# batra-mlp-lab/visdial

Measured on AMD Instinct MI355X. Metric: QA-rounds/sec training mn-att-ques-im-hist+disc (batch 20x10x100), higher is better.
Workload: dtype f32 operands and results; the option recurrence multiplies the EXACT 3-way bf16 split of both operands (9 bf16 MFMA products per fp32 product, f32 accumulate: fp32-grade, errors at the f32 MFMA's own level) -- its two step kernels and its weight-gradient contraction; f32 MFMA (v_mfma_f32_32x32x2_f32

## Files before the change

### visdial_amd/csrc/gemm_core.h

```cpp
#pragma once
#include <stdint.h>
#include <stdlib.h>
#include <type_traits>

#include "common.h"

#ifdef VD_TIMING
#define VD_TSLOTS 12
#define VD_TBLOCKS 8192
static __device__ unsigned long long vd_tbuf[VD_TBLOCKS * VD_TSLOTS];
#define VD_TSTAMP(i, clk)                                                                \
  do {                                                                                   \
    if (threadIdx.x == 0 && blockIdx.x < VD_TBLOCKS) vd_tbuf[blockIdx.x * VD_TSLOTS + (i)] = (clk); \
  } while (0)
#define VD_T(i) VD_TSTAMP(i, __builtin_amdgcn_s_memtime())
#define VD_TREAL(i) VD_TSTAMP(i, __builtin_amdgcn_s_memrealtime())
#else
#define VD_T(i) do {} while (0)
#define VD_TREAL(i) do {} while (0)
#endif

template <int WM_, int WK_, int NT_, int KW_, int DB_ = 1, int MINW_ = 1, int LDSMIN_ = 0, int BF16_ = 0>
struct GemmCfg {
  static constexpr int WM = WM_, WK = WK_, NT = NT_, KW = KW_, DB = DB_, MINW = MINW_;
  static constexpr int BM = WM * 32, BN = NT * 32, BK = WK * KW;
  static constexpr int THREADS = WM * WK * 64;
  static constexpr int BF16 = BF16_;
  static constexpr int ELEM_BYTES = BF16 ? 2 : 4;
  static constexpr int STRIDE = BF16 ? BK + 8 : BK + 4;
  static constexpr int BUF_FLOATS = (BM + BN) * STRIDE;
  static constexpr int STAGE_BYTES = (DB == 1 ? 2 : 1) * BUF_FLOATS * ELEM_BYTES;
  static constexpr int RED_BYTES = (WK - 1) * WM * 16 * 64 * 4;
  static constexpr int EPI_BYTES = WM * 32 * 32 * 4;
  static constexpr int LDS_BYTES0 = STAGE_BYTES > RED_BYTES ? STAGE_BYTES : RED_BYTES;
  static constexpr int LDS_BYTES1 = LDS_BYTES0 > EPI_BYTES ? LDS_BYTES0 : EPI_BYTES;
  static constexpr int LDS_BYTES = LDS_BYTES1 > LDSMIN_ ? LDS_BYTES1 : LDSMIN_;
  static constexpr int NA = (BM * BK / 4) / THREADS;
  static constexpr int NB = (BN * BK / 4) / THREADS;
  static_assert(KW % 8 == 0, "KW must be a multiple of 8");
  static_assert(!BF16 || (KW % 16 == 0 && DB == 0), "bf16 tiles: 16 k per MFMA, single-buffer pipeline only");
  static_assert((BM * BK / 4) % THREADS == 0 && NA >= 1, "A tile must split evenly");
  static_assert((BN * BK / 4) % THREADS == 0 && NB >= 1, "B tile must split evenly");
  static_assert(LDS_BYTES <= 160 * 1024, "LDS budget");
};

struct SrcRow {
  static constexpr bool KMAJOR = false;
  static constexpr bool PLAIN = true;
  const float* p;
  long ld;
  __device__ __forceinline__ const float* ptr(int r, int k) const { return p + (long)r * ld + k; }
  __device__ __forceinline__ long kstep() const { return 1; }
  __device__ __forceinline__ float4 ld4(int r, int k) const {
    return *reinterpret_cast<const float4*>(p + (long)r * ld + k);
  }
};
struct SrcK {
  static constexpr bool KMAJOR = true;
  static constexpr bool PLAIN = true;
  const float* p;
  long ld;
  __device__ __forceinline__ const float* ptr(int r, int k) const { return p + (long)k * ld + r; }
  __device__ __forceinline__ long kstep() const { return ld; }
  __device__ __forceinline__ float4 ld4(int r, int k) const {
    return *reinterpret_cast<const float4*>(p + (long)k * ld + r);
  }
};
struct SrcKRows {
  static constexpr bool KMAJOR = true;
  static constexpr bool PLAIN = false;
  const float* p;
  long ld;
  const int* rows;
  __device__ __forceinline__ float4 ld4(int r, int k) const {
    return *reinterpret_cast<const float4*>(p + (long)rows[k] * ld + r);
  }
};
struct SrcKGate4 {
  static constexpr bool KMAJOR = true;
  static constexpr bool PLAIN = true;
  const float* p;
  long ld;
  int H;
  __device__ __forceinline__ const float* ptr(int vc, int k) const {
    const int jb = vc >> 7, g = (vc >> 5) & 3, jj = vc & 31;
    return p + (long)k * ld + g * H + jb * 32 + jj;
  }
  __device__ __forceinline__ long kstep() const { return ld; }
  __device__ __forceinline__ float4 ld4(int vc, int k) const {
    const int jb = vc >> 7, g = (vc >> 5) & 3, jj = vc & 31;
    return *reinterpret_cast<const float4*>(p + (long)k * ld + g * H + jb * 32 + jj);
  }
};

__device__ __forceinline__ int mfma_row(int r, int lane) {
  return (r & 3) + 8 * (r >> 2) + 4 * (lane >> 5);
}

__device__ __forceinline__ void tile_to_rows(const f32x16& a, float* scr, int lane, float4 (&out)[4]) {
  asm volatile("" ::: "memory");
#pragma unroll
  for (int r = 0; r < 16; ++r) scr[mfma_row(r, lane) * 32 + (lane & 31)] = a[r];
  asm volatile("" ::: "memory");
#pragma unroll
  for (int p = 0; p < 4; ++p)
    out[p] = *reinterpret_cast<const float4*>(scr + (p * 8 + (lane >> 3)) * 32 + (lane & 7) * 4);
  asm volatile("" ::: "memory");
}

struct EpiNoPre {};
template <class Epi, class = void>
struct EpiPreOf {
  static constexpr bool value = false;
  using type = EpiNoPre;
};
template <class Epi>
struct EpiPreOf<Epi, std::void_t<typename Epi::Pre>> {
  static constexpr bool value = true;
  using type = typename Epi::Pre;
};

template <class Epi, class = void>
struct EpiDistOf {
  static constexpr bool value = false;
};
template <class Epi>
struct EpiDistOf<Epi, std::void_t<typename Epi::DOps>> {
  static constexpr bool value = Epi::HAS_DIST;
};

template <class Epi, class = void>
struct EpiDeadOf {
  static constexpr bool value = false;
};
template <class Epi>
struct EpiDeadOf<Epi, std::void_t<decltype(Epi::HAS_DEAD)>> {
  static constexpr bool value = Epi::HAS_DEAD;
};

template <class Epi, class = void>
struct EpiARowsOf {
  static constexpr bool value = false;
};
template <class Epi>
struct EpiARowsOf<Epi, std::void_t<decltype(Epi::HAS_AROWS)>> {
  static constexpr bool value = Epi::HAS_AROWS;
};

__device__ __forceinline__ void live_tile(int bid, int tiles_n, int& tile_m, int& tile_n) {
  const int li = bid >> 3;
  tile_m = (li / tiles_n) * 8 + (bid & 7);
  tile_n = li % tiles_n;
}

__device__ __forceinline__ int xcd_remap(int bid, int nwg) {
  const int q = nwg >> 3, r = nwg & 7;
  const int xcd = bid & 7, li = bid >> 3;
  const int base = xcd < r ? xcd * (q + 1) : r * (q + 1) + (xcd - r) * q;
  return base + li;
}

template <int D, int BK>
__device__ __forceinline__ void kmaj_piece(int f, int& r4, int& kk) {
  if constexpr (BK % 16 == 0) {
    const int klo = f & 15, g = f >> 4;
    r4 = g % (D / 4);
    kk = (g / (D / 4)) * 16 + klo;
    return;
  }
  const int klo = f & 7, g = f >> 3;
  r4 = g % (D / 4);
  kk = (g / (D / 4)) * 8 + klo;
}

template <class Cfg, class ASrc, class BSrc, class Epi>
__device__ __forceinline__ void gemm_block(int M, int N, int ks, int ke, int row_base, int col_base, int rot_seed,
                                           const ASrc& asrc, const BSrc& bsrc, const Epi& epi, float* smem,
                                           int tid_in = -1) {
  constexpr int WM = Cfg::WM, NT = Cfg::NT, KW = Cfg::KW;
  constexpr int BM = Cfg::BM, BN = Cfg::BN, BK = Cfg::BK;
  constexpr int THREADS = Cfg::THREADS, STR = Cfg::STRIDE;
  constexpr int NA = Cfg::NA, NB = Cfg::NB;
  const int tid = tid_in >= 0 ? tid_in : (int)threadIdx.x, lane = tid & 63, wave = tid >> 6;
  const int wm = wave % WM, wk = wave / WM;
  const int nk = ke > ks ? (ke - ks + BK - 1) / BK : 0;

  VD_T(0);
  VD_TREAL(6);
  f32x16 acc[NT];
#pragma unroll
  for (int j = 0; j < NT; ++j)
#pragma unroll
    for (int r = 0; r < 16; ++r) acc[j][r] = 0.f;

  float4 ra[NA], rb[NB];
  float4 ra2[NA], rb2[NB];

  const float* pa[NA];
  const float* pb[NB];
  int ka[NA], kb[NB];
  if constexpr (ASrc::PLAIN) {
#pragma unroll
    for (int i = 0; i < NA; ++i) {
      const int f = tid + i * THREADS;
      int gr;
      if constexpr (!ASrc::KMAJOR) {
        gr = row_base + f / (BK / 4);
        ka[i] = (f % (BK / 4)) * 4;
      } else {
        int r4;
        kmaj_piece<BM, BK>(f, r4, ka[i]);
        gr = row_base + r4 * 4;
      }
      pa[i] = gr < M ? asrc.ptr(gr, ka[i]) : nullptr;
    }
  }
  if constexpr (BSrc::PLAIN) {
#pragma unroll
    for (int i = 0; i < NB; ++i) {
      const int f = tid + i * THREADS;
      int gr;
      if constexpr (!BSrc::KMAJOR) {
        gr = col_base + f / (BK / 4);
        kb[i] = (f % (BK / 4)) * 4;
      } else {
        int r4;
        kmaj_piece<BN, BK>(f, r4, kb[i]);
        gr = col_base + r4 * 4;
      }
      pb[i] = gr < N ? bsrc.ptr(gr, kb[i]) : nullptr;
    }
  }

  auto load_tile_into = [&](int k0, float4 (&ra)[NA], float4 (&rb)[NB]) {
    if constexpr (ASrc::PLAIN) {
      const long off = (long)k0 * asrc.kstep();
#pragma unroll
      for (int i = 0; i < NA; ++i)
        ra[i] = (pa[i] != nullptr && k0 + ka[i] < ke) ? *reinterpret_cast<const float4*>(pa[i] + off)
                                                      : make_float4(0.f, 0.f, 0.f, 0.f);
    } else {
#pragma unroll
    for (int i = 0; i < NA; ++i) {
      const int f = tid + i * THREADS;
      float4 v = make_float4(0.f, 0.f, 0.f, 0.f);
      if constexpr (!ASrc::KMAJOR) {
        const int r = f / (BK / 4), kq = f % (BK / 4);
        const int gr = row_base + r, gk = k0 + kq * 4;
        if (gr < M && gk < ke) v = asrc.ld4(gr, gk);
      } else {
        int r4, kk;
        kmaj_piece<BM, BK>(f, r4, kk);
        const int gr = row_base + r4 * 4, gk = k0 + kk;
        if (gr < M && gk < ke) v = asrc.ld4(gr, gk);
      }
      ra[i] = v;
    }
    }
    if constexpr (BSrc::PLAIN) {
      const long off = (long)k0 * bsrc.kstep();
#pragma unroll
      for (int i = 0; i < NB; ++i)
        rb[i] = (pb[i] != nullptr && k0 + kb[i] < ke) ? *reinterpret_cast<const float4*>(pb[i] + off)
                                                      : make_float4(0.f, 0.f, 0.f, 0.f);
    } else {
#pragma unroll
    for (int i = 0; i < NB; ++i) {
      const int f = tid + i * THREADS;
      float4 v = make_float4(0.f, 0.f, 0.f, 0.f);
      if constexpr (!BSrc::KMAJOR) {
        const int r = f / (BK / 4), kq = f % (BK / 4);
        const int gr = col_base + r, gk = k0 + kq * 4;
        if (gr < N && gk < ke) v = bsrc.ld4(gr, gk);
      } else {
        int r4, kk;
        kmaj_piece<BN, BK>(f, r4, kk);
        const int gr = col_base + r4 * 4, gk = k0 + kk;
        if (gr < N && gk < ke) v = bsrc.ld4(gr, gk);
      }
      rb[i] = v;
    }
    }
  };

  auto load_tile = [&](int k0) { load_tile_into(k0, ra, rb); };

  using elem_t = std::conditional_t<Cfg::BF16 != 0, __bf16, float>;
  typedef __bf16 bf16x4_t __attribute__((ext_vector_type(4)));
  typedef __bf16 bf16x8_t __attribute__((ext_vector_type(8)));
  elem_t* const smem_e = reinterpret_cast<elem_t*>(smem);
  auto put_row4 = [&](elem_t* d, const float4& v) {
    if constexpr (Cfg::BF16) {
      bf16x4_t t = {(__bf16)v.x, (__bf16)v.y, (__bf16)v.z, (__bf16)v.w};
      *reinterpret_cast<bf16x4_t*>(d) = t;
    } else {
      *reinterpret_cast<float4*>(d) = v;
    }
  };
  auto put_col4 = [&](elem_t* d, const float4& v) {
    d[0] = (elem_t)v.x;
    d[STR] = (elem_t)v.y;
    d[2 * STR] = (elem_t)v.z;
    d[3 * STR] = (elem_t)v.w;
  };
  auto store_tile_from = [&](int buf, const float4 (&ra)[NA], const float4 (&rb)[NB]) {
    elem_t* sa = smem_e + buf * Cfg::BUF_FLOATS;
    elem_t* sb = sa + BM * STR;
#pragma unroll
    for (int i = 0; i < NA; ++i) {
      const int f = tid + i * THREADS;
      if constexpr (!ASrc::KMAJOR) {
        const int r = f / (BK / 4), kq = f % (BK / 4);
        put_row4(sa + r * STR + kq * 4, ra[i]);
      } else {
        int r4, kk;
        kmaj_piece<BM, BK>(f, r4, kk);
        put_col4(sa + (r4 * 4) * STR + kk, ra[i]);
      }
    }
#pragma unroll
    for (int i = 0; i < NB; ++i) {
      const int f = tid + i * THREADS;
      if constexpr (!BSrc::KMAJOR) {
        const int r = f / (BK / 4), kq = f % (BK / 4);
        put_row4(sb + r * STR + kq * 4, rb[i]);
      } else {
        int r4, kk;
        kmaj_piece<BN, BK>(f, r4, kk);
        put_col4(sb + (r4 * 4) * STR + kk, rb[i]);
      }
    }
  };

  const int rot = (rot_seed >= 0 && nk > 1) ? rot_seed % nk : 0;
  auto ktile = [&](int kt) {
    int t = kt + rot;
    if (t >= nk) t -= nk;
    return ks + t * BK;
  };
  auto store_tile = [&](int buf) { store_tile_from(buf, ra, rb); };

  const int frag_off = (lane & 31) * STR + wk * KW + (lane >> 5) * (Cfg::BF16 ? 8 : 4);
  auto mfma_tile = [&](int buf) {
    const elem_t* sa = smem_e + buf * Cfg::BUF_FLOATS + (wm * 32) * STR + frag_off;
    const elem_t* sb = smem_e + buf * Cfg::BUF_FLOATS + BM * STR + frag_off;
    if constexpr (Cfg::BF16) {
#pragma unroll
      for (int kc = 0; kc < KW / 16; ++kc) {
        const bf16x8_t a8 = *reinterpret_cast<const bf16x8_t*>(sa + kc * 16);
        bf16x8_t b8[NT];
#pragma unroll
        for (int j = 0; j < NT; ++j) b8[j] = *reinterpret_cast<const bf16x8_t*>(sb + j * 32 * STR + kc * 16);
#pragma unroll
        for (int j = 0; j < NT; ++j) acc[j] = __builtin_amdgcn_mfma_f32_32x32x16_bf16(a8, b8[j], acc[j], 0, 0, 0);
      }
    } else {
#pragma unroll
      for (int kc = 0; kc < KW / 8; ++kc) {
        const float4 a4 = *reinterpret_cast<const float4*>(sa + kc * 8);
        float4 b4[NT];
#pragma unroll
        for (int j = 0; j < NT; ++j) b4[j] = *reinterpret_cast<const float4*>(sb + j * 32 * STR + kc * 8);
#pragma unroll
        for (int j = 0; j < NT; ++j) acc[j] = __builtin_amdgcn_mfma_f32_32x32x2f32(a4.x, b4[j].x, acc[j], 0, 0, 0);
#pragma unroll
        for (int j = 0; j < NT; ++j) acc[j] = __builtin_amdgcn_mfma_f32_32x32x2f32(a4.y, b4[j].y, acc[j], 0, 0, 0);
#pragma unroll
        for (int j = 0; j < NT; ++j) acc[j] = __builtin_amdgcn_mfma_f32_32x32x2f32(a4.z, b4[j].z, acc[j], 0, 0, 0);
#pragma unroll
        for (int j = 0; j < NT; ++j) acc[j] = __builtin_amdgcn_mfma_f32_32x32x2f32(a4.w, b4[j].w, acc[j], 0, 0, 0);
      }
    }
  };

  if constexpr (Cfg::DB == 2) {
    if (nk > 0) load_tile_into(ktile(0), ra, rb);
    if (nk > 1) load_tile_into(ktile(1), ra2, rb2);
    for (int kt = 0; kt < nk; kt += 2) {
      store_tile_from(0, ra, rb);
      __syncthreads();
      if (kt == 0) VD_T(1);
      if (kt + 2 < nk) load_tile_into(ktile(kt + 2), ra, rb);
      mfma_tile(0);
      __syncthreads();
      if (kt + 1 < nk) {
        store_tile_from(0, ra2, rb2);
        __syncthreads();
        if (kt + 3 < nk) load_tile_into(ktile(kt + 3), ra2, rb2);
        mfma_tile(0);
        __syncthreads();
      }
    }
    VD_T(2);
  } else if constexpr (Cfg::DB == 1) {
    if (nk > 0) {
      load_tile(ktile(0));
      store_tile(0);
    }
    __syncthreads();
    for (int kt = 0; kt < nk; ++kt) {
      const int cur = kt & 1;
      if (kt + 1 < nk) load_tile(ktile(kt + 1));
      mfma_tile(cur);
      if (kt + 1 < nk) store_tile(cur ^ 1);
      __syncthreads();
    }
  } else {
    if (nk > 0) load_tile(ktile(0));
    for (int kt = 0; kt < nk; ++kt) {
      store_tile(0);
// ... 658 lines not shown
```

### visdial_amd/csrc/split_core.h

```cpp
#pragma once
#include "gemm_core.h"
#include "paths.h"

typedef __bf16 vd_bf16x8 __attribute__((ext_vector_type(8)));
typedef float vd_f32x4 __attribute__((ext_vector_type(4)));

__device__ __forceinline__ void vd_split3(const float4& u, const float4& w, vd_bf16x8& hi, vd_bf16x8& mid, vd_bf16x8& lo) {
  const float v[8] = {u.x, u.y, u.z, u.w, w.x, w.y, w.z, w.w};
#pragma unroll
  for (int i = 0; i < 8; ++i) {
    const __bf16 h = (__bf16)v[i];
    const float r1 = v[i] - (float)h;
    const __bf16 m = (__bf16)r1;
    const float r2 = r1 - (float)m;
    hi[i] = h; mid[i] = m; lo[i] = (__bf16)r2;
  }
}

static __global__ void __launch_bounds__(256) f32_to_bf16x3_kernel(const float* __restrict__ src, vd_bf16_bits* __restrict__ dst, long n4, long plane) {
  const long i = (long)blockIdx.x * 256 + threadIdx.x;
  if (i >= n4) return;
  const float4 v = reinterpret_cast<const float4*>(src)[i];
  float4 r1, r2;
  typedef __bf16 bf4 __attribute__((ext_vector_type(4)));
  const bf4 h = {(__bf16)v.x, (__bf16)v.y, (__bf16)v.z, (__bf16)v.w};
  r1.x = v.x - (float)h[0]; r1.y = v.y - (float)h[1]; r1.z = v.z - (float)h[2]; r1.w = v.w - (float)h[3];
  const bf4 m = {(__bf16)r1.x, (__bf16)r1.y, (__bf16)r1.z, (__bf16)r1.w};
  r2.x = r1.x - (float)m[0]; r2.y = r1.y - (float)m[1]; r2.z = r1.z - (float)m[2]; r2.w = r1.w - (float)m[3];
  const bf4 l = {(__bf16)r2.x, (__bf16)r2.y, (__bf16)r2.z, (__bf16)r2.w};
  *reinterpret_cast<bf4*>(dst + i * 4) = h;
  *reinterpret_cast<bf4*>(dst + plane + i * 4) = m;
  *reinterpret_cast<bf4*>(dst + 2 * plane + i * 4) = l;
}
static int weights_to_bf16x3(const float* src, vd_bf16_bits* dst, long n, hipStream_t s) {
  hipLaunchKernelGGL(f32_to_bf16x3_kernel, dim3((unsigned)((n / 4 + 255) / 256)), dim3(256), 0, s, src, dst, n / 4, n);
  VD_LAUNCH_CHECK();
  return VD_OK;
}

struct SplitCfg {
  static constexpr int NT = 4, WM = 4, THREADS = 256;
  static constexpr int BM = 128, BN = 128;
  static constexpr int ATILE = BM * 64;
  static constexpr int BTILE = BN * 32;
  static constexpr int STAGE = ATILE + 3 * BTILE;
#ifndef VD_SPLIT_LDS
#define VD_SPLIT_LDS 41984
#endif
  static constexpr int LDS_BYTES = VD_SPLIT_LDS;
  static_assert(LDS_BYTES >= 2 * STAGE, "two stages of 20 KB");
};

#ifndef VD_SPLIT_CG
#define VD_SPLIT_CG 2
#endif
static_assert(VD_SPLIT_CG >= 1 && VD_SPLIT_CG <= 8 && 8 % VD_SPLIT_CG == 0, "the XCD grid is VD_SPLIT_CG x (8 / VD_SPLIT_CG)");
__device__ __forceinline__ bool split_tile_of(int bid, int nwg, int tiles_m, int tiles_n, int& tile_m, int& tile_n) {
  constexpr int CG = VD_SPLIT_CG, RG = 8 / CG;
  if ((tiles_n % CG) == 0 && tiles_n >= 8) {
    const int xcd = bid & 7, li = bid >> 3, cpg = tiles_n / CG, rpg = (tiles_m + RG - 1) / RG;
    tile_n = (xcd % CG) * cpg + li % cpg;
    tile_m = (xcd / CG) * rpg + li / cpg;
    return tile_m < tiles_m && li / cpg < rpg;
  }
  const int wg = xcd_remap(bid, nwg);
  tile_n = wg % tiles_n;
  tile_m = wg / tiles_n;
  return true;
}
static int split_grid(int tiles_m, int tiles_n) {
  constexpr int CG = VD_SPLIT_CG, RG = 8 / CG;
  if ((tiles_n % CG) == 0 && tiles_n >= 8) return 8 * ((tiles_m + RG - 1) / RG) * (tiles_n / CG);
  return tiles_m * tiles_n;
}

template <int NPROD, class Epi>
__global__ void __launch_bounds__(256, 3)
gemm_split_kernel(int M, int N, int K, int tiles_n, const float* A, long lda, const vd_bf16_bits* B, long ldb, long bplane, Epi epi) {
  using Cfg = SplitCfg;
  constexpr int NT = Cfg::NT;
  extern __shared__ __attribute__((aligned(16))) float smem[];
  int tile_m, tile_n;
  if (!split_tile_of((int)blockIdx.x, (int)gridDim.x, (M + Cfg::BM - 1) / Cfg::BM, tiles_n, tile_m, tile_n)) return;
  const int row_base = tile_m * Cfg::BM, col_base = tile_n * Cfg::BN;
  constexpr int NIA = 2;
  constexpr int NIB = 3;
  const int tid = (int)threadIdx.x, lane = tid & 63;
  const int wm = __builtin_amdgcn_readfirstlane(tid >> 6);
  const int nm = K / 16;
  const int wrow = row_base + wm * 32;

  f32x16 acc[NT];
#pragma unroll
  for (int j = 0; j < NT; ++j)
#pragma unroll
    for (int r = 0; r < 16; ++r) acc[j][r] = 0.f;

  typename EpiPreOf<Epi>::type pre;
  if constexpr (EpiPreOf<Epi>::value) epi.preload(pre, wrow, lane, M);

  unsigned voffa[NIA], voffb[NIB];
#pragma unroll
  for (int i = 0; i < NIA; ++i) {
    const int r = wm * 32 + i * 16 + (lane >> 2);
    const int c = (lane & 3) ^ ((r >> 2) & 3);
    voffa[i] = (unsigned)(((long)min(row_base + r, M - 1) * lda + c * 4) * 4);
  }
  {
    const int r = wm * 32 + (lane >> 1);
    const int c = (lane & 1) ^ ((r >> 4) & 1);
    const unsigned v = (unsigned)(((long)min(col_base + r, N - 1) * ldb + c * 8) * 2);
#pragma unroll
    for (int i = 0; i < NIB; ++i) voffb[i] = v;
  }
  const unsigned lds0 = (unsigned)(uintptr_t)smem;
  auto issue = [&](int m, int st) {
    const unsigned base = lds0 + st * Cfg::STAGE;
#pragma unroll
    for (int i = 0; i < NIB; ++i)
      glds16(voffb[i], reinterpret_cast<const float*>(B + (long)i * bplane + (long)m * 16), base + Cfg::ATILE + i * Cfg::BTILE + wm * 1024);
    const float* ak = A + (long)m * 16;
#pragma unroll
    for (int i = 0; i < NIA; ++i) glds16(voffa[i], ak, base + (wm * NIA + i) * 1024);
  };
  const int hi = lane >> 5, l31 = lane & 31;
  const int sw = (l31 >> 2) & 3;
  const int cb = (hi ^ ((l31 >> 4) & 1)) * 16;

  if (nm > 0) {
    issue(0, 0);
    int st = 0;
    for (int m = 0; m < nm; ++m) {
      if (m + 1 < nm) {
        issue(m + 1, st ^ 1);
        asm volatile("s_waitcnt vmcnt(5)" ::: "memory");
      } else {
        asm volatile("s_waitcnt vmcnt(0)" ::: "memory");
      }
      asm volatile("s_barrier" ::: "memory");
      const char* sbase = reinterpret_cast<const char*>(smem) + st * Cfg::STAGE;
      const float* sa = reinterpret_cast<const float*>(sbase) + (wm * 32 + l31) * 16;
      const float4 u = *reinterpret_cast<const float4*>(sa + (((hi * 2) ^ sw) * 4));
      const float4 w = *reinterpret_cast<const float4*>(sa + (((hi * 2 + 1) ^ sw) * 4));
      vd_bf16x8 ap[3];
      vd_split3(u, w, ap[0], ap[1], ap[2]);
#pragma unroll
      for (int p = 2; p >= 0; --p) {
        vd_bf16x8 bp[NT];
#pragma unroll
        for (int j = 0; j < NT; ++j) {
          const vd_f32x4 t = *reinterpret_cast<const vd_f32x4*>(sbase + Cfg::ATILE + p * Cfg::BTILE + (j * 32 + l31) * 32 + cb);
          bp[j] = __builtin_bit_cast(vd_bf16x8, t);
        }
#pragma unroll
        for (int i = 2; i >= 0; --i) {
          constexpr int LIM = NPROD >= 9 ? 4 : NPROD >= 6 ? 2 : NPROD >= 3 ? 1 : 0;
          if (i + p > LIM) continue;
#pragma unroll
          for (int j = 0; j < NT; ++j) acc[j] = __builtin_amdgcn_mfma_f32_32x32x16_bf16(ap[i], bp[j], acc[j], 0, 0, 0);
        }
      }
      asm volatile("s_waitcnt lgkmcnt(0)\n\ts_barrier" ::: "memory");
      st ^= 1;
    }
  }
  if constexpr (EpiPreOf<Epi>::value) epi(acc, wrow, col_base, lane, M, N, smem + wm * 1024, &pre);
  else epi(acc, wrow, col_base, lane, M, N, smem + wm * 1024);
}

template <int NPROD, class Epi>
static int launch_gemm_split(int M, int N, int K, const float* A, long lda, const vd_bf16_bits* B, long ldb, long bplane, const Epi& e,
                             hipStream_t stream) {
  if (M <= 0 || N <= 0) return VD_OK;
  using Cfg = SplitCfg;
  VD_CHECK_ARG(K % 16 == 0 && lda % 4 == 0 && ldb % 8 == 0 && (long)M * lda * 4 < (1L << 32) && (long)N * ldb * 2 < (1L << 32),
               "launch_gemm_split: unsupported shape M=%d N=%d K=%d", M, N, K);
  const int tiles_m = vd_cdiv(M, Cfg::BM), tiles_n = vd_cdiv(N, Cfg::BN);
  auto kern = gemm_split_kernel<NPROD, Epi>;
  static bool attr_set = false;
  if (!attr_set) {
    VD_HIP(hipFuncSetAttribute(reinterpret_cast<const void*>(kern), hipFuncAttributeMaxDynamicSharedMemorySize, 160 * 1024));
    attr_set = true;
  }
  hipLaunchKernelGGL(kern, dim3(split_grid(tiles_m, tiles_n)), dim3(256), Cfg::LDS_BYTES, stream, M, N, K, tiles_n, A, lda, B, ldb, bplane, e);
  VD_LAUNCH_CHECK();
  return VD_OK;
}

template <class Epi>
static int launch_gemm_split(int nprod, int M, int N, int K, const float* A, long lda, const vd_bf16_bits* B, long ldb, long bplane,
                             const Epi& e, hipStream_t stream) {
  if (nprod == 9) return launch_gemm_split<9>(M, N, K, A, lda, B, ldb, bplane, e, stream);
  if (nprod == 6) return launch_gemm_split<6>(M, N, K, A, lda, B, ldb, bplane, e, stream);
  return launch_gemm_split<3>(M, N, K, A, lda, B, ldb, bplane, e, stream);
}

struct SplitTnCfg {
  static constexpr int BM = 256, BN = 128, THREADS = 256;
  static constexpr int ATILE = 16 * BM * 4;
  static constexpr int BTILE = 16 * BN * 4;
  static constexpr int STAGE = ATILE + BTILE;
  static constexpr int LDS_BYTES = 2 * STAGE;
};
static_assert(SplitTnCfg::BM == VD_SPLIT_TN_BM && SplitTnCfg::BN == VD_SPLIT_TN_BN, "paths.h vd_tn_split_tiles");

template <int NPROD>
__global__ void __launch_bounds__(256, 2)
gemm_split_tn_kernel(int M, int N, int kchunk, int K, int tiles, int tiles_n, int splits, const float* A, long lda, const float* B, long ldb,
                     float* C, long ldc) {
  using Cfg = SplitTnCfg;
  extern __shared__ __attribute__((aligned(16))) float smem[];
  int tile, split;
  if ((splits & 7) == 0) {
    const int xcd = (int)blockIdx.x & 7, li = (int)blockIdx.x >> 3;
    split = xcd * (splits >> 3) + li / tiles;
    tile = li % tiles;
  } else {
    split = (int)blockIdx.x / tiles;
    tile = (int)blockIdx.x % tiles;
  }
  const int m_base = (tile / tiles_n) * Cfg::BM, n_base = (tile % tiles_n) * Cfg::BN;
  const int ks = split * kchunk, ke = min(K, ks + kchunk);
  const int nm = ke > ks ? (ke - ks) / 16 : 0;
  const int tid = (int)threadIdx.x, lane = tid & 63;
  const int wm = __builtin_amdgcn_readfirstlane(tid >> 6);

  f32x16 acc[2][4];
#pragma unroll
  for (int mb = 0; mb < 2; ++mb)
#pragma unroll
    for (int j = 0; j < 4; ++j)
#pragma unroll
      for (int r = 0; r < 16; ++r) acc[mb][j][r] = 0.f;

  unsigned voffa[4], voffb[2];
#pragma unroll
  for (int i = 0; i < 4; ++i) voffa[i] = (unsigned)(((long)(wm * 4 + i) * lda + m_base + lane * 4) * 4);
#pragma unroll
  for (int i = 0; i < 2; ++i) voffb[i] = (unsigned)(((long)((wm * 2 + i) * 2 + (lane >> 5)) * ldb + n_base + (lane & 31) * 4) * 4);
  const unsigned lds0 = (unsigned)(uintptr_t)smem;
  auto issue = [&](int m, int st) {
    const unsigned base = lds0 + st * Cfg::STAGE;
    const float* ak = A + (long)(ks + m * 16) * lda;
    const float* bk = B + (long)(ks + m * 16) * ldb;
#pragma unroll
    for (int i = 0; i < 2; ++i) glds16(voffb[i], bk, base + Cfg::ATILE + (wm * 2 + i) * 1024);
#pragma unroll
    for (int i = 0; i < 4; ++i) glds16(voffa[i], ak, base + (wm * 4 + i) * 1024);
  };
  const int hi = lane >> 5, l31 = lane & 31;

  if (nm > 0) {
    issue(0, 0);
    int st = 0;
    for (int m = 0; m < nm; ++m) {
      if (m + 1 < nm) {
        issue(m + 1, st ^ 1);
        asm volatile("s_waitcnt vmcnt(6)" ::: "memory");
      } else {
        asm volatile("s_waitcnt vmcnt(0)" ::: "memory");
      }
      asm volatile("s_barrier" ::: "memory");
      const float* sA = reinterpret_cast<const float*>(reinterpret_cast<const char*>(smem) + st * Cfg::STAGE) + (hi * 8) * Cfg::BM + wm * 64 + l31;
      const float* sB = reinterpret_cast<const float*>(reinterpret_cast<const char*>(smem) + st * Cfg::STAGE + Cfg::ATILE) + (hi * 8) * Cfg::BN + l31;
      vd_bf16x8 ap[2][3], bp[2][3];
      auto load_b = [&](int j, vd_bf16x8 (&dst)[3]) {
        const float* p = sB + j * 32;
        const float4 u = make_float4(p[0], p[Cfg::BN], p[2 * Cfg::BN], p[3 * Cfg::BN]);
        const float4 w = make_float4(p[4 * Cfg::BN], p[5 * Cfg::BN], p[6 * Cfg::BN], p[7 * Cfg::BN]);
        vd_split3(u, w, dst[0], dst[1], dst[2]);
      };
#pragma unroll
      for (int mb = 0; mb < 2; ++mb) {
        const float* p = sA + mb * 32;
        const float4 u = make_float4(p[0], p[Cfg::BM], p[2 * Cfg::BM], p[3 * Cfg::BM]);
        const float4 w = make_float4(p[4 * Cfg::BM], p[5 * Cfg::BM], p[6 * Cfg::BM], p[7 * Cfg::BM]);
        vd_split3(u, w, ap[mb][0], ap[mb][1], ap[mb][2]);
      }
      load_b(0, bp[0]);
#pragma unroll
      for (int j = 0; j < 4; ++j) {
        __builtin_amdgcn_sched_barrier(0);
        if (j + 1 < 4) load_b(j + 1, bp[(j + 1) & 1]);
#pragma unroll
        for (int pb = 2; pb >= 0; --pb)
#pragma unroll
          for (int pa = 2; pa >= 0; --pa) {
            constexpr int LIM = NPROD >= 9 ? 4 : NPROD >= 6 ? 2 : NPROD >= 3 ? 1 : 0;
            if (pa + pb > LIM) continue;
#pragma unroll
            for (int mb = 0; mb < 2; ++mb) acc[mb][j] = __builtin_amdgcn_mfma_f32_32x32x16_bf16(ap[mb][pa], bp[j & 1][pb], acc[mb][j], 0, 0, 0);
          }
        if (j + 1 < 4) {
          __builtin_amdgcn_sched_group_barrier(0x100, 4, 0);
#pragma unroll
          for (int i = 0; i < 18; ++i) {
            __builtin_amdgcn_sched_group_barrier(0x008, 1, 0);
            __builtin_amdgcn_sched_group_barrier(0x002, 4, 0);
          }
        }
      }
      asm volatile("s_waitcnt lgkmcnt(0)\n\ts_barrier" ::: "memory");
      st ^= 1;
    }
  }
  if (nm == 0) return;
  const EpiAtomic<4> e{C, ldc};
#pragma unroll
  for (int mb = 0; mb < 2; ++mb) e(acc[mb], m_base + wm * 64 + mb * 32, n_base, lane, M, N);
}

template <int NPROD>
static int launch_gemm_split_tn(int M, int N, int K, const float* A, long lda, const float* B, long ldb, float* C, long ldc, hipStream_t stream) {
  using Cfg = SplitTnCfg;
  VD_CHECK_ARG(M % Cfg::BM == 0 && N % Cfg::BN == 0 && K % 16 == 0 && lda % 4 == 0 && ldb % 4 == 0 && 16L * lda * 4 < (1L << 31) && 16L * ldb * 4 < (1L << 31),
               "launch_gemm_split_tn: unsupported shape M=%d N=%d K=%d", M, N, K);
  if (K == 0) return VD_OK;
  const int tiles_n = N / Cfg::BN, tiles = (M / Cfg::BM) * tiles_n;
  int splits = vd_cdiv(2L * vd_num_cus(), tiles);
  splits = (splits + 7) & ~7;
  int kchunk = vd_cdiv(vd_cdiv(K, splits), 16) * 16;
  if (kchunk < 64) kchunk = 64;
  splits = vd_cdiv(K, kchunk);
  if (splits >= 8) splits = (splits + 7) & ~7;
  auto kern = gemm_split_tn_kernel<NPROD>;
  static bool attr_set = false;
  if (!attr_set) {
    VD_HIP(hipFuncSetAttribute(reinterpret_cast<const void*>(kern), hipFuncAttributeMaxDynamicSharedMemorySize, 160 * 1024));
    attr_set = true;
  }
  hipLaunchKernelGGL(kern, dim3(tiles * splits), dim3(256), Cfg::LDS_BYTES, stream, M, N, kchunk, K, tiles, tiles_n, splits, A, lda, B, ldb, C, ldc);
  VD_LAUNCH_CHECK();
  return VD_OK;
}
```

Measured before the change: 8794.

## Restructure split GEMM to 16x16x32 bf16 MFMA with K=32 stages and register A loads

Rewrites the 3-way bf16 split GEMM kernel to use 16x16x32 MFMA instructions over a K=32 step per stage instead of 32x32x16 over K=16. This halves the number of barrier-synchronised iterations. A is now loaded directly from global memory into registers and split in registers, so only the three B planes go through LDS via async copies. Accumulators are converted back to the 32x32 tile layout through an LDS scratch shuffle before the unchanged epilogue, which adds epilogue work and LDS use. It also handles a K%32 remainder of 16 with a masked tail.

```diff
diff --git a/visdial_amd/csrc/gemm_core.h b/visdial_amd/csrc/gemm_core.h
--- a/visdial_amd/csrc/gemm_core.h
+++ b/visdial_amd/csrc/gemm_core.h
@@ -106,6 +106,28 @@
   for (int p = 0; p < 4; ++p)
     out[p] = *reinterpret_cast<const float4*>(scr + (p * 8 + (lane >> 3)) * 32 + (lane & 7) * 4);
   asm volatile("" ::: "memory");
+}
+
+typedef float vd_f32x4 __attribute__((ext_vector_type(4)));
+constexpr int QUAD_LD = 36;
+__device__ __forceinline__ int quad_row(int i, int lane) { return 4 * (lane >> 4) + i; }
+__device__ __forceinline__ f32x16 quad_to_tile(const vd_f32x4& q00, const vd_f32x4& q01, const vd_f32x4& q10, const vd_f32x4& q11, float* scr,
+                                               int lane) {
+  asm volatile("" ::: "memory");
+#pragma unroll
+  for (int i = 0; i < 4; ++i) {
+    float* w = scr + quad_row(i, lane) * QUAD_LD + (lane & 15);
+    w[0] = q00[i];
+    w[16] = q01[i];
+    w[16 * QUAD_LD] = q10[i];
+    w[16 * QUAD_LD + 16] = q11[i];
+  }
+  asm volatile("" ::: "memory");
+  f32x16 t;
+#pragma unroll
+  for (int r = 0; r < 16; ++r) t[r] = scr[mfma_row(r, lane) * QUAD_LD + (lane & 31)];
+  asm volatile("" ::: "memory");
+  return t;
 }
 
 struct EpiNoPre {};
diff --git a/visdial_amd/csrc/split_core.h b/visdial_amd/csrc/split_core.h
--- a/visdial_amd/csrc/split_core.h
+++ b/visdial_amd/csrc/split_core.h
@@ -3,7 +3,6 @@
 #include "paths.h"
 
 typedef __bf16 vd_bf16x8 __attribute__((ext_vector_type(8)));
-typedef float vd_f32x4 __attribute__((ext_vector_type(4)));
 
 __device__ __forceinline__ void vd_split3(const float4& u, const float4& w, vd_bf16x8& hi, vd_bf16x8& mid, vd_bf16x8& lo) {
   const float v[8] = {u.x, u.y, u.z, u.w, w.x, w.y, w.z, w.w};
@@ -39,16 +38,13 @@
 }
 
 struct SplitCfg {
-  static constexpr int NT = 4, WM = 4, THREADS = 256;
-  static constexpr int BM = 128, BN = 128;
-  static constexpr int ATILE = BM * 64;
-  static constexpr int BTILE = BN * 32;
-  static constexpr int STAGE = ATILE + 3 * BTILE;
-#ifndef VD_SPLIT_LDS
-#define VD_SPLIT_LDS 41984
-#endif
-  static constexpr int LDS_BYTES = VD_SPLIT_LDS;
-  static_assert(LDS_BYTES >= 2 * STAGE, "two stages of 20 KB");
+    static constexpr int NT = 4, WM = 4, THREADS = 64 * WM;
+  static constexpr int BM = 32 * WM, BN = 128, KS = 32;
+  static constexpr int BTILE = BN * 64;
+  static constexpr int STAGE = 3 * BTILE;
+  static constexpr int LDS_BYTES = 2 * STAGE;
+  static constexpr int SCR = LDS_BYTES / WM / 4;
+  static_assert(SCR >= 32 * QUAD_LD, "quad_to_tile's 32 rows of QUAD_LD floats");
 };
 
 #ifndef VD_SPLIT_CG
@@ -68,6 +64,7 @@
   tile_m = wg / tiles_n;
   return true;
 }
+__device__ __forceinline__ int split_swz(int q) { return (0x78 >> (2 * (q & 3))) & 3; }
 static int split_grid(int tiles_m, int tiles_n) {
   constexpr int CG = VD_SPLIT_CG, RG = 8 / CG;
   if ((tiles_n % CG) == 0 && tiles_n >= 8) return 8 * ((tiles_m + RG - 1) / RG) * (tiles_n / CG);
@@ -75,7 +72,7 @@
 }
 
 template <int NPROD, class Epi>
-__global__ void __launch_bounds__(256, 3)
+__global__ void __launch_bounds__(SplitCfg::THREADS, 3)
 gemm_split_kernel(int M, int N, int K, int tiles_n, const float* A, long lda, const vd_bf16_bits* B, long ldb, long bplane, Epi epi) {
   using Cfg = SplitCfg;
   constexpr int NT = Cfg::NT;
@@ -83,73 +80,79 @@
   int tile_m, tile_n;
   if (!split_tile_of((int)blockIdx.x, (int)gridDim.x, (M + Cfg::BM - 1) / Cfg::BM, tiles_n, tile_m, tile_n)) return;
   const int row_base = tile_m * Cfg::BM, col_base = tile_n * Cfg::BN;
-  constexpr int NIA = 2;
-  constexpr int NIB = 3;
+  constexpr int NIB = 24 / Cfg::WM;
   const int tid = (int)threadIdx.x, lane = tid & 63;
   const int wm = __builtin_amdgcn_readfirstlane(tid >> 6);
-  const int nm = K / 16;
+  const int nfull = K / 32, nm = nfull + ((K >> 4) & 1);
   const int wrow = row_base + wm * 32;
-
-  f32x16 acc[NT];
-#pragma unroll
-  for (int j = 0; j < NT; ++j)
-#pragma unroll
-    for (int r = 0; r < 16; ++r) acc[j][r] = 0.f;
+  const int g = lane >> 4, l15 = lane & 15;
+
+  vd_f32x4 acc[2][2 * NT];
+#pragma unroll
+  for (int rt = 0; rt < 2; ++rt)
+#pragma unroll
+    for (int j = 0; j < 2 * NT; ++j)
+#pragma unroll
+      for (int r = 0; r < 4; ++r) acc[rt][j][r] = 0.f;
 
   typename EpiPreOf<Epi>::type pre;
   if constexpr (EpiPreOf<Epi>::value) epi.preload(pre, wrow, lane, M);
 
-  unsigned voffa[NIA], voffb[NIB];
-#pragma unroll
-  for (int i = 0; i < NIA; ++i) {
-    const int r = wm * 32 + i * 16 + (lane >> 2);
-    const int c = (lane & 3) ^ ((r >> 2) & 3);
-    voffa[i] = (unsigned)(((long)min(row_base + r, M - 1) * lda + c * 4) * 4);
-  }
-  {
-    const int r = wm * 32 + (lane >> 1);
-    const int c = (lane & 1) ^ ((r >> 4) & 1);
-    const unsigned v = (unsigned)(((long)min(col_base + r, N - 1) * ldb + c * 8) * 2);
-#pragma unroll
-    for (int i = 0; i < NIB; ++i) voffb[i] = v;
+  unsigned aoff[2];
+#pragma unroll
+  for (int rt = 0; rt < 2; ++rt) aoff[rt] = (unsigned)(((long)min(wrow + rt * 16 + l15, M - 1) * lda + g * 8) * 4);
+  float4 an[2][2];
+  auto load_a = [&](int m) {
+    const char* ak = reinterpret_cast<const char*>(A + (long)m * 32);
+    const bool live = m < nfull || g < 2;
+#pragma unroll
+    for (int rt = 0; rt < 2; ++rt) {
+      an[rt][0] = an[rt][1] = make_float4(0.f, 0.f, 0.f, 0.f);
+      if (live) {
+        an[rt][0] = *reinterpret_cast<const float4*>(ak + aoff[rt]);
+        an[rt][1] = *reinterpret_cast<const float4*>(ak + aoff[rt] + 16);
+      }
+    }
+  };
+  const int csrc = (lane & 3) ^ split_swz(lane >> 4);
+  unsigned voffb[NIB];
+#pragma unroll
+  for (int i = 0; i < NIB; ++i) {
+    const int r = ((wm * NIB + i) & 7) * 16 + (lane >> 2);
+    voffb[i] = (unsigned)(((long)min(col_base + r, N - 1) * ldb + csrc * 8) * 2);
   }
   const unsigned lds0 = (unsigned)(uintptr_t)smem;
-  auto issue = [&](int m, int st) {
-    const unsigned base = lds0 + st * Cfg::STAGE;
-#pragma unroll
-    for (int i = 0; i < NIB; ++i)
-      glds16(voffb[i], reinterpret_cast<const float*>(B + (long)i * bplane + (long)m * 16), base + Cfg::ATILE + i * Cfg::BTILE + wm * 1024);
-    const float* ak = A + (long)m * 16;
-#pragma unroll
-    for (int i = 0; i < NIA; ++i) glds16(voffa[i], ak, base + (wm * NIA + i) * 1024);
+  auto issue_b = [&](int m, int st) {
+    const unsigned back = m < nfull ? 0u : (unsigned)(csrc >> 1) * 32u;
+#pragma unroll
+    for (int i = 0; i < NIB; ++i) {
+      const int q = wm * NIB + i;
+      glds16(voffb[i] - back, reinterpret_cast<const float*>(B + (long)(q >> 3) * bplane + (long)m * 32), lds0 + st * Cfg::STAGE + q * 1024);
+    }
   };
-  const int hi = lane >> 5, l31 = lane & 31;
-  const int sw = (l31 >> 2) & 3;
-  const int cb = (hi ^ ((l31 >> 4) & 1)) * 16;
+  const int bfrag = l15 * 64 + ((g ^ split_swz(l15 >> 2)) * 16);
 
   if (nm > 0) {
-    issue(0, 0);
+    issue_b(0, 0);
+    load_a(0);
     int st = 0;
     for (int m = 0; m < nm; ++m) {
+      vd_bf16x8 ap[2][3];
+#pragma unroll
+      for (int rt = 0; rt < 2; ++rt) vd_split3(an[rt][0], an[rt][1], ap[rt][0], ap[rt][1], ap[rt][2]);
+      asm volatile("s_waitcnt vmcnt(0)" ::: "memory");
+      asm volatile("s_barrier" ::: "memory");
       if (m + 1 < nm) {
-        issue(m + 1, st ^ 1);
-        asm volatile("s_waitcnt vmcnt(5)" ::: "memory");
-      } else {
-        asm volatile("s_waitcnt vmcnt(0)" ::: "memory");
-      }
-      asm volatile("s_barrier" ::: "memory");
-      const char* sbase = reinterpret_cast<const char*>(smem) + st * Cfg::STAGE;
-      const float* sa = reinterpret_cast<const float*>(sbase) + (wm * 32 + l31) * 16;
-      const float4 u = *reinterpret_cast<const float4*>(sa + (((hi * 2) ^ sw) * 4));
-      const float4 w = *reinterpret_cast<const float4*>(sa + (((hi * 2 + 1) ^ sw) * 4));
-      vd_bf16x8 ap[3];
-      vd_split3(u, w, ap[0], ap[1], ap[2]);
+        issue_b(m + 1, st ^ 1);
+        load_a(m + 1);
+      }
+      const char* sbase = reinterpret_cast<const char*>(smem) + st * Cfg::STAGE + bfrag;
 #pragma unroll
       for (int p = 2; p >= 0; --p) {
-        vd_bf16x8 bp[NT];
-#pragma unroll
-        for (int j = 0; j < NT; ++j) {
-          const vd_f32x4 t = *reinterpret_cast<const vd_f32x4*>(sbase + Cfg::ATILE + p * Cfg::BTILE + (j * 32 + l31) * 32 + cb);
+        vd_bf16x8 bp[2 * NT];
+#pragma unroll
+        for (int j = 0; j < 2 * NT; ++j) {
+          const vd_f32x4 t = *reinterpret_cast<const vd_f32x4*>(sbase + p * Cfg::BTILE + j * 1024);
           bp[j] = __builtin_bit_cast(vd_bf16x8, t);
         }
 #pragma unroll
@@ -157,15 +160,21 @@
           constexpr int LIM = NPROD >= 9 ? 4 : NPROD >= 6 ? 2 : NPROD >= 3 ? 1 : 0;
           if (i + p > LIM) continue;
 #pragma unroll
-          for (int j = 0; j < NT; ++j) acc[j] = __builtin_amdgcn_mfma_f32_32x32x16_bf16(ap[i], bp[j], acc[j], 0, 0, 0);
+          for (int rt = 0; rt < 2; ++rt)
+#pragma unroll
+            for (int j = 0; j < 2 * NT; ++j) acc[rt][j] = __builtin_amdgcn_mfma_f32_16x16x32_bf16(ap[rt][i], bp[j], acc[rt][j], 0, 0, 0);
         }
       }
       asm volatile("s_waitcnt lgkmcnt(0)\n\ts_barrier" ::: "memory");
       st ^= 1;
     }
   }
-  if constexpr (EpiPreOf<Epi>::value) epi(acc, wrow, col_base, lane, M, N, smem + wm * 1024, &pre);
-  else epi(acc, wrow, col_base, lane, M, N, smem + wm * 1024);
+  float* scr = smem + wm * Cfg::SCR;
+  f32x16 tile[NT];
+#pragma unroll
+  for (int j = 0; j < NT; ++j) tile[j] = quad_to_tile(acc[0][2 * j], acc[0][2 * j + 1], acc[1][2 * j], acc[1][2 * j + 1], scr, lane);
+  if constexpr (EpiPreOf<Epi>::value) epi(tile, wrow, col_base, lane, M, N, scr, &pre);
+  else epi(tile, wrow, col_base, lane, M, N, scr);
 }
 
 template <int NPROD, class Epi>
@@ -182,7 +191,7 @@
     VD_HIP(hipFuncSetAttribute(reinterpret_cast<const void*>(kern), hipFuncAttributeMaxDynamicSharedMemorySize, 160 * 1024));
     attr_set = true;
   }
-  hipLaunchKernelGGL(kern, dim3(split_grid(tiles_m, tiles_n)), dim3(256), Cfg::LDS_BYTES, stream, M, N, K, tiles_n, A, lda, B, ldb, bplane, e);
+  hipLaunchKernelGGL(kern, dim3(split_grid(tiles_m, tiles_n)), dim3(Cfg::THREADS), Cfg::LDS_BYTES, stream, M, N, K, tiles_n, A, lda, B, ldb, bplane, e);
   VD_LAUNCH_CHECK();
   return VD_OK;
 }
```

Result: faster. 9160 (median of 6 runs) (+4.2%).
